# sloisel/MultiGridBarrier.jl

Measured on AMD Instinct MI355X. Metric: Newton iters/sec + wall-clock to converge, 2D P2 p-Laplace L=9, higher is better.
Workload: dtype f64

## Files before the change

multigridbarrier.jl_amd/csrc/mf_big_inv.hpp:

```cpp
#pragma once
#include "mf_device.hpp"

namespace mgbhip {
namespace {

constexpr int BIGI_THREADS = 1024;

#include "ldlt32.hpp"

__device__ __forceinline__ void block_ldlt32(double (*Dn)[NB + 1], double* dq, int nb, int tid, int32_t* __restrict__ status) {
    block_ldlt32_mfma(Dn, dq, nb, tid, status);
}
__device__ __forceinline__ void block_inverse32_sel(const double (*Ls)[NB + 1], double (*Wv)[NB + 1], double (*Tm)[17], int tid) {
    block_inverse32_mfma(Ls, Wv, Tm, tid);
}

__device__ __forceinline__ void block0_to_slot(double (*Dn)[NB + 1], double (*Wv)[NB + 1], double (*Tm)[17], double* dq, int nb,
                                               int tid, int32_t* __restrict__ status, double* __restrict__ slot) {
    block_ldlt32(Dn, dq, nb, tid, status);
    block_inverse32_sel(Dn, Wv, Tm, tid);
    for (int i = tid; i < NB * NB; i += 256) {
        const int rr = i % NB, c = i / NB;
        if (rr >= c && rr < nb) slot[rr + NB * c] = (rr == c) ? dq[rr] : Wv[rr][c];
    }
}

__device__ __forceinline__ void slice_transform(double (*P)[ST + 1], double (*Pout)[ST + 1], double (*P2)[ST + 1],
                                                const double (*Wv)[NB + 1], const double* rd, int lane, int wave) {
    const int fr = lane & 15, fk = lane >> 4;
    const int rr = 16 * wave + fr;
    double4_t acc0 = {0.0, 0.0, 0.0, 0.0}, acc1 = {0.0, 0.0, 0.0, 0.0};
#pragma unroll
    for (int kk = 0; kk < NB / 4; ++kk) {
        const double a = P[4 * kk + fk][rr];
        if (kk < 4) acc0 = __builtin_amdgcn_mfma_f64_16x16x4f64(Wv[fr][4 * kk + fk], a, acc0, 0, 0, 0);
        acc1 = __builtin_amdgcn_mfma_f64_16x16x4f64(Wv[16 + fr][4 * kk + fk], a, acc1, 0, 0, 0);
    }
#pragma unroll
    for (int r = 0; r < 4; ++r) {
        const int q0 = fk + 4 * r, q1 = 16 + fk + 4 * r;
        Pout[q0][rr] = acc0[r];
        Pout[q1][rr] = acc1[r];
        if (P2) {
            P2[q0][rr] = acc0[r] * rd[q0];
            P2[q1][rr] = acc1[r] * rd[q1];
        }
    }
}

#ifdef MGB_STEP_PROBE
#define PROBE(i) do { __builtin_amdgcn_sched_barrier(0); __builtin_amdgcn_s_waitcnt(0); if (is_la && blockIdx.y == 0 && tid == 0 && j0 == 64 && gridDim.y == 1 && F.k > 400) g_probe[i] = wall_clock64(); if (!is_la && blockIdx.x == 0 && blockIdx.y == 0 && tid == 0 && j0 == 64 && gridDim.y == 1 && F.k > 400) g_probe[16 + i] = wall_clock64(); __builtin_amdgcn_s_waitcnt(0); __builtin_amdgcn_sched_barrier(0); } while (0)
#else
#define PROBE(i) do { } while (0)
#endif

__global__ __launch_bounds__(256, 3) void mf_big_step(const FrontDev* __restrict__ fr, int32_t first, int j0,
                                                   double* __restrict__ arena, double* __restrict__ dscr,
                                                   double* __restrict__ dvec, int32_t* __restrict__ status,
                                                   int do_diag) {
    __shared__ double Wv[NB][NB + 1];
    __shared__ double Dn[NB][NB + 1];
    __shared__ double Tm[16][17];
    __shared__ double dq[NB], rdq[NB];
    __shared__ double Pa[NB][ST + 1];
    __shared__ double Pb[NB][ST + 1];
    const FrontDev F = fr[first + blockIdx.y];
    const int m = F.m, k = F.k;
    if (j0 >= k) return;
    const int nb = min(NB, k - j0);
    const int j1 = j0 + nb;
    const int T = (m - j1 + ST - 1) / ST;
    const int tid = threadIdx.x, lane = tid & 63, wave = tid >> 6;
    double* W = arena + F.F_off;
    double* slot = dscr + ((int64_t)blockIdx.y * 2 + ((j0 / NB) & 1)) * (NB * NB);
    const bool is_la = blockIdx.x == gridDim.x - 1;
    int ti = 0, tj = 0;
    if (!is_la) {
        const int lin = blockIdx.x;
        ti = (int)((sqrt(8.0 * lin + 1.0) - 1.0) * 0.5);
        while ((ti + 1) * (ti + 2) / 2 <= lin) ++ti;
        while (ti * (ti + 1) / 2 > lin) --ti;
        tj = lin - ti * (ti + 1) / 2;
        if (ti >= T) return;
    }
    const bool look = j1 < k;
    const int nbn = look ? min(NB, k - j1) : 0;
    const int rbase = is_la ? j1 : j1 + ti * ST, cbase = j1 + tj * ST;
    PROBE(0);
#ifdef MGB_STEP_PROBE
    if (is_la && blockIdx.y == 0 && tid == 0 && j0 == 64 && gridDim.y == 1 && F.k > 400) g_probe[34] = clock64();
#endif
    const int fr16 = lane & 15, fk = lane >> 4;

    double pa[NB * ST / 256], pb[NB * ST / 256];
#pragma unroll
    for (int u = 0; u < NB * ST / 256; ++u) {
        const int i = tid + 256 * u, rr = i % ST, q = i / ST;
        const int r = rbase + rr, c = cbase + rr;
        const bool rin = is_la ? (rr < nbn) : (r < m);
        pa[u] = (q < nb && rin) ? W[r + (int64_t)(j0 + q) * m] : 0.0;
        pb[u] = (!is_la && ti != tj && q < nb && c < m) ? W[c + (int64_t)(j0 + q) * m] : 0.0;
    }
    double cw[4][4];
    if (!is_la) {
#pragma unroll
        for (int tb = 0; tb < 4; ++tb)
#pragma unroll
            for (int r = 0; r < 4; ++r) {
                const int row = rbase + 16 * wave + fr16, col = cbase + 16 * tb + fk + 4 * r;
                cw[tb][r] = (row < m && col < m && row >= col) ? W[row + (int64_t)col * m] : 0.0;
            }
    } else {
#pragma unroll
        for (int t = 0; t < 4; ++t) {
            const int i = tid + 256 * t, rr = i % NB, c = i / NB;
            cw[0][t] = (look && rr >= c && rr < nbn) ? W[(j1 + rr) + (int64_t)(j1 + c) * m] : 0.0;
        }
    }
    if (do_diag) {
        for (int i = tid; i < NB * NB; i += 256) {
            const int rr = i % NB, c = i / NB;
            Dn[rr][c] = (rr >= c && rr < nb) ? W[(j0 + rr) + (int64_t)(j0 + c) * m] : 0.0;
        }
        __syncthreads();
        block_ldlt32(Dn, dq, nb, tid, is_la ? status : nullptr);
        block_inverse32_sel(Dn, Wv, Tm, tid);
    } else {
        for (int i = tid; i < NB * NB; i += 256) {
            const int rr = i % NB, c = i / NB;
            const double v = (rr >= c && rr < nb) ? slot[rr + NB * c] : 0.0;
            Wv[rr][c] = (rr > c) ? v : (rr == c ? 1.0 : 0.0);
            if (rr == c) dq[rr] = (rr < nb) ? v : 1.0;
        }
    }
#pragma unroll
    for (int u = 0; u < NB * ST / 256; ++u) {
        const int i = tid + 256 * u, rr = i % ST, q = i / ST;
        Pa[q][rr] = pa[u];
        Pb[q][rr] = pb[u];
    }
    __syncthreads();
    PROBE(1);
    if (tid < NB) rdq[tid] = 1.0 / dq[tid];
    if (is_la ? T == 0 : blockIdx.x == 0) {
        {
            const int rt = wave & 1, ct = wave >> 1;
            if (ct <= rt) {
                double4_t accm = {0.0, 0.0, 0.0, 0.0};
#pragma unroll
                for (int kk = 0; kk < NB / 4; ++kk) {
                    const int kq = 4 * kk + fk;
                    accm = __builtin_amdgcn_mfma_f64_16x16x4f64(kq < nb ? Wv[kq][16 * ct + fr16] / dq[kq] : 0.0, Wv[kq][16 * rt + fr16], accm, 0, 0, 0);
                }
#pragma unroll
                for (int r = 0; r < 4; ++r) {
                    const int row = 16 * rt + fr16, col = 16 * ct + fk + 4 * r;
                    if (row < nb && col < row) W[(j0 + col) + (int64_t)(j0 + row) * m] = accm[r];
                    else if (row < nb && col == row) dvec[F.idx_off + j0 + row] = accm[r];
                }
            }
        }
    }
    if (is_la && !look) return;
    __syncthreads();
    PROBE(2);
    if (is_la) {
        if (wave < 2) slice_transform(Pa, Pa, Pb, Wv, rdq, lane, wave);
        __syncthreads();
        PROBE(3);
        {
            const int rt = wave & 1, ct = wave >> 1;
            double4_t accd = {0.0, 0.0, 0.0, 0.0};
#pragma unroll
            for (int kk = 0; kk < NB / 4; ++kk)
                accd = __builtin_amdgcn_mfma_f64_16x16x4f64(Pb[4 * kk + fk][16 * ct + fr16], Pa[4 * kk + fk][16 * rt + fr16],
                                                            accd, 0, 0, 0);
#pragma unroll
            for (int r = 0; r < 4; ++r) {
                const int rr = 16 * rt + fr16, c = 16 * ct + fk + 4 * r;
                Dn[rr][c] = -accd[r];
            }
        }
        __syncthreads();
#pragma unroll
        for (int t = 0; t < 4; ++t) {
            const int i = tid + 256 * t, rr = i % NB, c = i / NB;
            Dn[rr][c] = (rr >= c && rr < nbn) ? cw[0][t] + Dn[rr][c] : 0.0;
        }
        __syncthreads();
        double* nslot = dscr + ((int64_t)blockIdx.y * 2 + ((j1 / NB) & 1)) * (NB * NB);
        PROBE(4);
#ifdef MGB_STEP_PROBE
        double sv[4];
        for (int t = 0; t < 4; ++t) { const int i = tid + 256 * t; sv[t] = Dn[i % NB][i / NB]; }
        __syncthreads();
        __builtin_amdgcn_sched_barrier(0);
        if (is_la && blockIdx.y == 0 && tid == 0 && j0 == 64 && gridDim.y == 1 && F.k > 400) { g_probe[32] = clock64(); g_probe[36] = wall_clock64(); }
        __builtin_amdgcn_sched_barrier(0);
        block_ldlt32(Dn, dq, nbn, tid, nullptr);
        __builtin_amdgcn_sched_barrier(0);
        if (is_la && blockIdx.y == 0 && tid == 0 && j0 == 64 && gridDim.y == 1 && F.k > 400) { g_probe[33] = clock64(); g_probe[37] = wall_clock64(); }
        __builtin_amdgcn_sched_barrier(0);
        for (int t = 0; t < 4; ++t) { const int i = tid + 256 * t; Dn[i % NB][i / NB] = sv[t]; }
        __syncthreads();
        __builtin_amdgcn_sched_barrier(0);
        if (is_la && blockIdx.y == 0 && tid == 0 && j0 == 64 && gridDim.y == 1 && F.k > 400) { g_probe[38] = clock64(); g_probe[44] = wall_clock64(); }
        __builtin_amdgcn_sched_barrier(0);
#endif
        block_ldlt32(Dn, dq, nbn, tid, status);
#ifdef MGB_STEP_PROBE
        __builtin_amdgcn_sched_barrier(0);
        if (is_la && blockIdx.y == 0 && tid == 0 && j0 == 64 && gridDim.y == 1 && F.k > 400) { g_probe[39] = clock64(); g_probe[45] = wall_clock64(); }
        __builtin_amdgcn_sched_barrier(0);
#endif
        PROBE(5);
        block_inverse32_sel(Dn, Wv, Tm, tid);
        PROBE(6);
        for (int i = tid; i < NB * NB; i += 256) {
            const int rr = i % NB, c = i / NB;
            if (rr >= c && rr < nbn) nslot[rr + NB * c] = (rr == c) ? dq[rr] : Wv[rr][c];
        }
        PROBE(7);
#ifdef MGB_STEP_PROBE
        if (is_la && blockIdx.y == 0 && tid == 0 && j0 == 64 && gridDim.y == 1 && F.k > 400) g_probe[35] = clock64();
#endif
        return;
    }
    if (ti == tj) {
        slice_transform(Pa, Pa, Pb, Wv, rdq, lane, wave);
    } else {
        slice_transform(Pa, Pa, nullptr, Wv, rdq, lane, wave);
        {
            const int rr = 16 * wave + fr16;
            double4_t acc0 = {0.0, 0.0, 0.0, 0.0}, acc1 = {0.0, 0.0, 0.0, 0.0};
#pragma unroll
            for (int kk = 0; kk < NB / 4; ++kk) {
                const double a = Pb[4 * kk + fk][rr];
                if (kk < 4) acc0 = __builtin_amdgcn_mfma_f64_16x16x4f64(Wv[fr16][4 * kk + fk], a, acc0, 0, 0, 0);
                acc1 = __builtin_amdgcn_mfma_f64_16x16x4f64(Wv[16 + fr16][4 * kk + fk], a, acc1, 0, 0, 0);
            }
#pragma unroll
            for (int r = 0; r < 4; ++r) {
                const int q0 = fk + 4 * r, q1 = 16 + fk + 4 * r;
                Pb[q0][rr] = acc0[r] * rdq[q0];
                Pb[q1][rr] = acc1[r] * rdq[q1];
            }
        }
    }
    __syncthreads();
    PROBE(3);
    double4_t acc[4];
#pragma unroll
    for (int tb = 0; tb < 4; ++tb) acc[tb] = double4_t{0.0, 0.0, 0.0, 0.0};
#pragma unroll
    for (int kk = 0; kk < NB / 4; ++kk) {
        const double s = Pa[4 * kk + fk][16 * wave + fr16];
#pragma unroll
        for (int tb = 0; tb < 4; ++tb) {
            if (ti == tj && tb > wave) continue;
            acc[tb] = __builtin_amdgcn_mfma_f64_16x16x4f64(Pb[4 * kk + fk][16 * tb + fr16], s, acc[tb], 0, 0, 0);
        }
    }
    const int nskip = (blockIdx.x == 0 && look) ? nbn : 0;
#pragma unroll
    for (int tb = 0; tb < 4; ++tb)
#pragma unroll
        for (int r = 0; r < 4; ++r) {
            const int row = rbase + 16 * wave + fr16, col = cbase + 16 * tb + fk + 4 * r;
            if (row < m && col < m && row >= col && !(row - j1 < nskip && col - j1 < nskip))
                W[row + (int64_t)col * m] = cw[tb][r] - acc[tb][r];
        }
    PROBE(4);
}

__global__ __launch_bounds__(256) void mf_tri_pack(int m, const double* __restrict__ F, double* __restrict__ packed, int unpack,
                                                   double* __restrict__ Fout) {
    const int c = blockIdx.x;
    if (c >= m) return;
    const int64_t base = (int64_t)c * m - ((int64_t)c * (c - 1)) / 2;
    for (int r = c + threadIdx.x; r < m; r += 256) {
        if (unpack) Fout[r + (int64_t)c * m] = packed[base + (r - c)];
        else packed[base + (r - c)] = F[r + (int64_t)c * m];
    }
}

__global__ __launch_bounds__(256) void mf_big_diag0(const FrontDev* __restrict__ fr, int32_t first,
                                                    const double* __restrict__ arena, double* __restrict__ dscr,
                                                    int32_t* __restrict__ status) {
    __shared__ double Wv[NB][NB + 1];
    __shared__ double Dn[NB][NB + 1];
    __shared__ double Tm[16][17];
    __shared__ double dq[NB];
    const FrontDev F = fr[first + blockIdx.x];
    const int m = F.m, nb = min(NB, F.k), tid = threadIdx.x;
    const double* W = arena + F.F_off;
    for (int i = tid; i < NB * NB; i += 256) {
        const int rr = i % NB, c = i / NB;
        Dn[rr][c] = (rr >= c && rr < nb) ? W[rr + (int64_t)c * m] : 0.0;
    }
    __syncthreads();
    block0_to_slot(Dn, Wv, Tm, dq, nb, tid, status, dscr + (int64_t)blockIdx.x * 2 * (NB * NB));
}

__global__ __launch_bounds__(BIGI_THREADS) void mf_fwd_inv(const FrontDev* __restrict__ fr, int32_t first,
                                                           const int32_t* __restrict__ front_idx,
                                                           const int64_t* __restrict__ ug_ptr,
                                                           const int64_t* __restrict__ ug_src,
                                                           const double* __restrict__ arena,
                                                           const double* __restrict__ dvec,
                                                           const double* __restrict__ b, double* __restrict__ y,
                                                           double* __restrict__ uvec) {
    extern __shared__ double sh[];
#ifdef MGB_STEP_PROBE
#define FP(i) do { if (threadIdx.x == 0 && gridDim.x > 150) { const long long _t = wall_clock64(); if (blockIdx.x == 0) g_probe[48 + i] = _t; if (i == 0) atomicMin((unsigned long long*)&g_probe[56], (unsigned long long)_t); if (i == 5) { atomicMax((unsigned long long*)&g_probe[57], (unsigned long long)_t); atomicAdd((unsigned long long*)&g_probe[58], (unsigned long long)(_t - g_probe[56])); } } } while (0)
#else
#define FP(i) do { } while (0)
#endif
    FP(0);
    const FrontDev F = fr[first + blockIdx.x];
    const int m = F.m, k = F.k;
    const int tid = threadIdx.x, nt = BIGI_THREADS;
    double* tl = sh;
    double* Ml = sh + ((m + 1) & ~1);
    double* uq = Ml + NB * (NB + 1);
    double* part = uq + 2 * NB;
    const int32_t* idx = front_idx + F.idx_off;
    const double* Fm = arena + F.F_off;
    const double* dv = dvec + F.idx_off;
    {
        const int64_t* up = ug_ptr + F.ug_off;
        for (int j = tid; j < m; j += nt) {
            double v = (j < k) ? b[idx[j]] : 0.0;
            const int64_t e1 = up[j + 1];
            for (int64_t e = up[j]; e < e1; e += 4) {
                double a[4];
#pragma unroll
                for (int u = 0; u < 4; ++u) a[u] = (e + u < e1) ? uvec[ug_src[e + u]] : 0.0;
#pragma unroll
                for (int u = 0; u < 4; ++u) v += a[u];
            }
            tl[j] = v;
        }
    }
    const int wa = tid % NB, wb = tid / NB;
    {
        const double w0 = (wa < wb && wb < k) ? Fm[wa + (int64_t)wb * m] : 0.0;
        if (wa < wb) { Ml[wb * (NB + 1) + wa] = w0; Ml[wa * (NB + 1) + wb] = w0; }
        if (tid < NB) Ml[tid * (NB + 1) + tid] = (tid < k) ? dv[tid] : 0.0;
    }
    __syncthreads();
    FP(1);
    for (int j0 = 0; j0 < k; j0 += NB) {
        const int nb = min(NB, k - j0), j1 = j0 + nb;
        const int jn = j0 + NB;
        const double wnext = (wa < wb && jn + wb < k) ? Fm[(jn + wa) + (int64_t)(jn + wb) * m] : 0.0;
// ... 219 lines not shown
                    }
                }
            }
        }
        {
            const int q = tid >> 5, c = tid & 31;
            double ph = Ml[q * (NB + 1) + c] * (c < nb ? gl[j0 + c] : 0.0);
            ph += quad_perm_f64<0xB1>(ph);
            ph += quad_perm_f64<0x4E>(ph);
            ph += quad_perm_f64<0x124>(ph);
            ph += quad_perm_f64<0x128>(ph);
            ph += __shfl_xor(ph, 16, 32);
            if (c == 0) zq[q] = (q < nb) ? tl[j0 + q] - ph : 0.0;
        }
        if (j0 == 256) BP(5);
        __syncthreads();
        if (j0 == 256) BP(6);
        if (tid < nb) x[il[j0 + tid]] = zq[tid];
        if (wa < wb) { Ml[wb * (NB + 1) + wa] = wnext; Ml[wa * (NB + 1) + wb] = wnext; }
        if (tid < NB) Ml[tid * (NB + 1) + tid] = dnext;
        double zr[8];
#pragma unroll
        for (int t = 0; t < 4; ++t) {
            zr[2 * t] = zq[2 * cp + 8 * t];
            zr[2 * t + 1] = zq[2 * cp + 8 * t + 1];
        }
#pragma unroll
        for (int ps = 0; ps < 2; ++ps) {
            const int q = cq + ps * CPP;
            if (q < j0) {
                double v = 0.0;
#pragma unroll
                for (int t = 0; t < 4; ++t) v += pa[ps][t].a * zr[2 * t] + pa[ps][t].b * zr[2 * t + 1];
                v += quad_perm_f64<0xB1>(v);
                v += quad_perm_f64<0x4E>(v);
                if (cp == 0) gl[q] += v;
            }
        }
        for (int q = cq + 2 * CPP; q - cq < j0; q += CPP) {
            const double* Aq = Fm + (int64_t)min(q, j0 - 1) * m + j0 + 2 * cp;
            D2 a[4];
#pragma unroll
            for (int t = 0; t < 4; ++t) {
                if (nb == NB) a[t] = *reinterpret_cast<const D2*>(Aq + 8 * t);
                else {
                    const int o = 2 * cp + 8 * t;
                    a[t].a = Aq[min(o, nb - 1) - 2 * cp];
                    a[t].b = Aq[min(o + 1, nb - 1) - 2 * cp];
                }
            }
            double v = 0.0;
#pragma unroll
            for (int t = 0; t < 4; ++t) v += a[t].a * zr[2 * t] + a[t].b * zr[2 * t + 1];
            v += quad_perm_f64<0xB1>(v);
            v += quad_perm_f64<0x4E>(v);
            if (cp == 0 && q < j0) gl[q] += v;
        }
        if (j0 == 256) BP(7);
        __syncthreads();
    }
    BP(9);
}

__global__ __launch_bounds__(BIGI_THREADS) void mf_bwd_inv(const FrontDev* __restrict__ fr, int32_t first,
                                                           const int32_t* __restrict__ front_idx,
                                                           const double* __restrict__ arena,
                                                           const double* __restrict__ dvec,
                                                           const double* __restrict__ y, double* __restrict__ x) {
    bwd_inv_front<false>(fr, first, blockIdx.x, front_idx, arena, dvec, y, x, nullptr, 0, nullptr);
}
__global__ __launch_bounds__(BIGI_THREADS) void mf_bwd_inv_split(const FrontDev* __restrict__ fr, int32_t first,
                                                                 const int32_t* __restrict__ front_idx,
                                                                 const double* __restrict__ arena,
                                                                 const double* __restrict__ dvec,
                                                                 const double* __restrict__ y, double* __restrict__ x,
                                                                 double* gscr, int gstride, uint32_t* cnt) {
    bwd_inv_front<true>(fr, first, blockIdx.y, front_idx, arena, dvec, y, x, gscr, gstride, cnt);
}

inline void launch_big_diag0(const FactorArgs& a, const MfLaunch& L, int nfronts) {
    hipLaunchKernelGGL(mf_big_diag0, dim3(nfronts), dim3(256), 0, a.st, a.fr, L.first, a.arena, a.dscr, a.status);
}
inline void launch_inv_steps(const FactorArgs& a, const MfLaunch& L, int nfronts, bool diag_in_step0) {
    for (int j0 = 0; j0 < L.max_k; j0 += NB) {
        const int rem = L.max_m - j0;
        const int T = std::max(0, (rem - 1 + ST - 1) / ST);
        const dim3 gs(T * (T + 1) / 2 + 1, nfronts);
        hipLaunchKernelGGL(mf_big_step, gs, dim3(256), 0, a.st, a.fr, L.first, j0, a.arena, a.dscr, a.dvec, a.status,
                           (j0 == 0 && diag_in_step0) ? 1 : 0);
    }
}

inline void launch_tri_pack(int m, double* F, double* packed, bool unpack, hipStream_t st) {
    hipLaunchKernelGGL(mf_tri_pack, dim3(m), dim3(256), 0, st, m, unpack ? (const double*)nullptr : F, packed, unpack ? 1 : 0,
                       unpack ? F : (double*)nullptr);
}

inline size_t fwd_inv_lds(int max_m) {
    return (size_t)(((max_m + 1) & ~1) + NB * (NB + 1) + 2 * NB + BIGI_THREADS) * sizeof(double);
}
inline size_t bwd_inv_lds(int max_m, int max_k) {
    return (size_t)(((max_m + 1) & ~1) + ((max_k + 1) & ~1) + NB * (NB + 1) + 2 * NB + (max_m + 1) / 2) * sizeof(double);
}
inline void launch_fwd_inv(const SolveArgs& a, const MfLaunch& L) {
    hipLaunchKernelGGL(mf_fwd_inv, dim3(L.count), dim3(BIGI_THREADS), fwd_inv_lds(L.max_m), a.st, a.fr, L.first, a.front_idx,
                       a.ug_ptr, a.ug_src, a.arena, a.dvec, a.b, a.y, a.uvec);
}
inline void launch_bwd_inv(const SolveArgs& a, const MfLaunch& L) {
    const int S = a.bwd_cnt ? bwd_inv_split(L.count, L.max_k, L.max_m) : 1;
    if (S > 1) {
        hipLaunchKernelGGL(mf_bwd_inv_split, dim3(S, L.count), dim3(BIGI_THREADS), bwd_inv_lds(L.max_m, L.max_k), a.st, a.fr, L.first,
                           a.front_idx, a.arena, a.dvec, a.y, a.x, a.bwd_g, (int)bwd_split_stride(L.max_k), a.bwd_cnt);
        return;
    }
    hipLaunchKernelGGL(mf_bwd_inv, dim3(L.count), dim3(BIGI_THREADS), bwd_inv_lds(L.max_m, L.max_k), a.st, a.fr, L.first,
                       a.front_idx, a.arena, a.dvec, a.y, a.x);
}

}
}
```

multigridbarrier.jl_amd/csrc/mf_launch_plan.hpp:

```cpp
#pragma once
#include <algorithm>
#include <cstdint>
#include <cstdlib>
#include <vector>

#include "host_util.hpp"
#include "mf_analysis.hpp"

namespace mgbhip {

struct MfLaunch {
    int32_t first, count;
    int32_t cls;
    int32_t max_m, max_k;
    int32_t max_child = 0;
    bool tiny = false;
    bool wave = false;
    bool inv = false;
    bool iface = false;
    int32_t grec_first = -1;
};

constexpr int BIG_INV_MAX_M = 7000;
constexpr int GATHER_MAX_CHILD = 8;
constexpr int BIG_DIAG0_MIN_COUNT = 24;

struct MfSwitches {
    bool no_geo;
    bool old_big;
    bool merge_groups;
    bool packed_leaves;
    bool wave_small;
    int64_t inv_min_n;
    int64_t wave_min_n;
    bool gather_lds_maps;
    int gather_ct;
    bool bwd_split;
    int small_threads;
    bool border_launches;
    static MfSwitches from_env() {
        auto num = [](const char* name, long long dflt) { const char* e = getenv(name); return e ? atoll(e) : dflt; };
        return {env_on("MGBHIP_NO_GEO"), env_on("MGBHIP_OLD_BIG"), !env_on("MGBHIP_NO_MERGE_GROUPS"), !env_on("MGBHIP_NO_PACKED_LEAVES"),
                !env_on("MGBHIP_NO_WAVE_SMALL"), num("MGBHIP_INV_MIN_N", 1024), num("MGBHIP_WAVE_MIN_N", 0),
                env_on("MGBHIP_GATHER_LDS_MAPS"), (int)num("MGBHIP_GATHER_CT", 0), num("MGBHIP_BWD_SPLIT", 1) != 0,
                (int)num("MGBHIP_SMALL_THREADS", 0), env_on("MGBHIP_BORDER_LAUNCHES")};
    }
};

using LevelLaunches = std::vector<std::vector<MfLaunch>>;

inline MfLaunch launch_of_range(const MfPlan& plan, MfLaunch L, int32_t first, int32_t count) {
    L.first = first; L.count = count;
    L.max_m = 0; L.max_k = 0; L.max_child = 0;
    for (int32_t t = first; t < first + count; ++t) {
        L.max_m = std::max(L.max_m, plan.fronts[t].m);
        L.max_k = std::max(L.max_k, plan.fronts[t].k);
        L.max_child = std::max(L.max_child, plan.fronts[t].nchild);
    }
    return L;
}

inline void merge_straggler_groups(const MfPlan& plan, std::vector<MfLaunch>& G) {
    auto absorb = [&](size_t into, size_t from) {
        MfLaunch& A = G[into];
        const MfLaunch& B = G[from];
        A.first = B.first;
        A.count += B.count;
        A.max_k = std::max(A.max_k, B.max_k);
        A.max_child = std::max(A.max_child, B.max_child);
        G.erase(G.begin() + (long)from);
    };
    if (G.size() >= 2 && G.back().cls == 0 && G.back().inv) {
        int64_t lds_count = 0;
        bool ok = true;
        for (size_t g = 0; g + 1 < G.size(); ++g) { lds_count += G[g].count; ok = ok && !G[g].tiny && plan.fronts[G[g].first].m > 32; }
        if (ok && lds_count <= G.back().count)
            while (G.size() >= 2) absorb(G.size() - 1, G.size() - 2);
    }
    for (size_t g = 0; g + 1 < G.size();) {
        const bool next_lds = G[g + 1].cls != 0;
        if (next_lds && !G[g].tiny && (G[g].count < 256 || 4 * (int64_t)G[g].count < G[g + 1].count)) absorb(g + 1, g);
        else ++g;
    }
}

inline void split_interface_front(const MfPlan& plan, LevelLaunches& levels, bool inv_allowed) {
    const int32_t q = plan.iface_front;
    for (auto& G : levels) {
        for (size_t g = 0; g < G.size(); ++g) {
            const MfLaunch L = G[g];
            if (q < L.first || q >= L.first + L.count) continue;
            std::vector<MfLaunch> out;
            if (q > L.first) out.push_back(launch_of_range(plan, L, L.first, q - L.first));
            MfLaunch I = launch_of_range(plan, L, q, 1);
            I.cls = 0; I.tiny = false; I.wave = false; I.iface = true;
            I.inv = (I.max_m <= BIG_INV_MAX_M && inv_allowed);
            out.push_back(I);
            if (q + 1 < L.first + L.count) out.push_back(launch_of_range(plan, L, q + 1, L.first + L.count - q - 1));
            G.erase(G.begin() + (long)g);
            G.insert(G.begin() + (long)g, out.begin(), out.end());
            break;
        }
    }
}

inline bool only_small_children(const MfPlan& plan, const MfLaunch& L) {
    for (int32_t q = L.first; q < L.first + L.count; ++q) {
        const Front& f = plan.fronts[q];
        for (int32_t c = 0; c < f.nchild; ++c) {
            const Front& ch = plan.fronts[plan.children[f.child_off + c]];
            if ((ch.m - ch.k) * (ch.m - ch.k) > 64) return false;
        }
    }
    return true;
}

inline LevelLaunches classify_launches(const MfPlan& plan, int32_t lds_cap, bool inv_ok, const MfSwitches& sw) {
    static const int32_t classes[] = {16, 32, 48, 64, 88, 128};
    const bool inv_allowed = inv_ok && !sw.old_big && plan.n >= sw.inv_min_n;
    const int32_t nlev = (int32_t)plan.level_ptr.size() - 1;
    LevelLaunches levels(nlev);
    for (int32_t l = 0; l < nlev; ++l) {
        int32_t i = plan.level_ptr[l];
        const int32_t end = plan.level_ptr[l + 1];
        while (i < end) {
            const int32_t m = plan.fronts[i].m;
            int32_t cls = 0;
            for (int32_t c : classes)
// ... 77 lines not shown
    return (L.iface || L.count >= BIG_DIAG0_MIN_COUNT) ? MF_B0_DIAG0 : MF_B0_STEP0;
}
inline int backward_small_kmax(const MfLaunch& L) { return L.max_k <= 8 ? 8 : (L.max_k <= 16 ? 16 : 0); }

inline size_t factor_small_lds(int cls) {
    return (size_t)((cls >= 88 ? cls * (cls + 1) / 2 : cls * cls) + 8 * cls) * sizeof(double);
}
constexpr int SMALL_STATIC_LDS = 2112;
constexpr int CU_LDS_BYTES = 160 * 1024;
constexpr int SMALL_FILL_WAVES = 24;
inline int factor_small_threads(const MfLaunch& L, int compute_units, int forced = 0) {
    if (L.cls <= 16) return 64;
    if (L.cls <= 32) return 128;
    if (forced == 256 || forced == 512 || forced == 1024) return forced;
    const int64_t cu = std::max(compute_units, 1);
    const int64_t fit = std::max<int64_t>(1, CU_LDS_BYTES / (int64_t)(factor_small_lds(L.cls) + SMALL_STATIC_LDS));
    const int64_t per_cu = std::min(fit, ((int64_t)L.count + cu - 1) / cu);
    int threads = 256;
    while (threads < 1024 && per_cu * (2 * threads / 64) <= SMALL_FILL_WAVES) threads *= 2;
    return threads;
}
static_assert(16 - 1 <= 64 && 32 - 1 <= 128 && 128 - 1 <= 256, "mf_factor_small solves one panel row per thread");

constexpr int GATHER_MIN_WGS = 768;
inline int big_gather_ct(const MfLaunch& L, int forced) {
    if (forced == 8 || forced == 16 || forced == 32) return forced;
    int ct = 8;
    while (ct < 32 && (int64_t)L.count * ((L.max_m + 2 * ct - 1) / (2 * ct)) >= GATHER_MIN_WGS) ct *= 2;
    return ct;
}

constexpr int BWD_SPLIT_MAX = 16;
constexpr int BWD_SPLIT_CUS = 256;
constexpr int BWD_SPLIT_COLS = 64;
constexpr int BWD_THIN_BOUNDARY = 8;
inline int bwd_inv_split(int32_t count, int32_t max_k, int32_t max_m) {
    if (count < 1 || max_m - max_k <= BWD_THIN_BOUNDARY) return 1;
    return std::max(1, std::min({BWD_SPLIT_MAX, BWD_SPLIT_CUS / count, (max_k + BWD_SPLIT_COLS - 1) / BWD_SPLIT_COLS}));
}
inline int32_t bwd_split_stride(int32_t max_k) { return (max_k + 1) & ~1; }
inline void bwd_split_scratch(const LevelLaunches& solves, int64_t out[2]) {
    out[0] = out[1] = 0;
    for (auto& lev : solves)
        for (auto& L : lev) {
            if (L.count == 0 || L.cls || !L.inv || bwd_inv_split(L.count, L.max_k, L.max_m) == 1) continue;
            out[0] = std::max<int64_t>(out[0], L.count);
            out[1] = std::max<int64_t>(out[1], (int64_t)L.count * bwd_split_stride(L.max_k));
        }
}

struct GatherRec {
    int64_t map_off;
    int64_t base[GATHER_MAX_CHILD];
    int32_t ld[GATHER_MAX_CHILD];
    int32_t bs[GATHER_MAX_CHILD];
};

inline void build_gather_maps(const MfPlan& plan, LevelLaunches& levels, std::vector<GatherRec>& recs, std::vector<int32_t>& gmap) {
    recs.clear();
    gmap.clear();
    for (auto& lev : levels)
        for (auto& L : lev) {
            L.grec_first = -1;
            if (L.count == 0 || big_assembly_kind(L) != MF_ASM_GATHER) continue;
            L.grec_first = (int32_t)recs.size();
            for (int32_t q = L.first; q < L.first + L.count; ++q) {
                const Front& f = plan.fronts[q];
                GatherRec R{};
                R.map_off = (int64_t)gmap.size();
                gmap.resize(gmap.size() + (size_t)f.nchild * (size_t)f.m, -1);
                for (int32_t c = 0; c < f.nchild; ++c) {
                    const Front& ch = plan.fronts[plan.children[f.child_off + c]];
                    R.base[c] = ch.F_off + (int64_t)ch.k * ch.m + ch.k;
                    R.ld[c] = ch.m;
                    R.bs[c] = ch.m - ch.k;
                    int32_t* mp = gmap.data() + R.map_off + (int64_t)c * f.m;
                    for (int32_t j = 0; j < ch.m - ch.k; ++j) mp[plan.rel[ch.rel_off + j]] = j;
                }
                recs.push_back(R);
            }
        }
}

constexpr int MF_LAUNCH_ROW = 16;
inline int64_t launch_rows(const LevelLaunches& levels, const LevelLaunches& solves, bool leaf_packed, bool robust,
                           int32_t* out, int64_t cap) {
    int64_t n = 0;
    for (size_t l = 0; l < levels.size(); ++l) {
        int32_t bwd = 0;
        for (auto& S : solves[l])
            if (S.cls && !S.tiny) { const int km = backward_small_kmax(S); bwd = km == 8 ? MF_BWD_K8 : (km == 16 ? MF_BWD_K16 : MF_BWD_GENERAL); }
        for (auto& L : levels[l]) {
            if (n < cap && out) {
                const bool inv = L.inv && !robust;
                int32_t* r = out + n * MF_LAUNCH_ROW;
                r[0] = (int32_t)l; r[1] = L.first; r[2] = L.count; r[3] = L.cls; r[4] = L.max_m; r[5] = L.max_k; r[6] = L.max_child;
                r[7] = L.tiny; r[8] = L.wave; r[9] = inv; r[10] = L.iface; r[11] = L.tiny && leaf_packed;
                r[12] = big_assembly_kind(L); r[13] = big_block0_kind(L, inv); r[14] = (L.cls && !L.tiny) ? bwd : (int32_t)MF_BWD_NA; r[15] = 0;
            }
            ++n;
        }
    }
    return n;
}

}
```

multigridbarrier.jl_amd/csrc/mf_numeric.hip:

```cpp
#include <hip/hip_runtime.h>

#include <cstdio>

#include <algorithm>
#include <cstdlib>

#include "../../include/mgbhip.h"
#include "mf_solver.hpp"
#include "mf_device.hpp"
#include "mf_small.hpp"
#include "mf_big_subst.hpp"
#include "mf_big_inv.hpp"
#include "mf_big_assemble.hpp"

namespace mgbhip {

namespace {

int32_t query_lds_cap() {
    if (hipFuncSetAttribute((const void*)mf_factor_small<8, true>, hipFuncAttributeMaxDynamicSharedMemorySize,
                            (int)factor_small_lds(128)) == hipSuccess)
        return 128;
    (void)hipGetLastError();
    return 88;
// ... 88 lines not shown
    static StageTimers& timers_or_dummy(StageTimers* t) {
        static const bool on = env_on("MGBHIP_LEVEL_TIMING");
        return (t && on) ? *t : g_dummy_timers;
    }
    LevelScope(StageTimers* t, const char* sweep, int level)
        : scope(timers_or_dummy(t), (snprintf(nm, sizeof(nm), "%s_lv%02d", sweep, level), nm)) {}
};

}

void MfSolver::upload_plan(hipStream_t st) {
    d_front_idx.upload(plan.front_idx, st);
    d_children.upload(plan.children, st);
    d_rel.upload(plan.rel, st);
    d_a_src.upload(plan.a_src, st);
    d_a_colptr.upload(plan.a_colptr, st);
    d_arena.alloc((size_t)std::max<int64_t>(plan.arena_doubles, 1));
    d_uvec.alloc((size_t)std::max<int64_t>(plan.uvec_doubles, 1));
    d_y.alloc((size_t)plan.n + 1);
    y_zero = y_border_one = status_zero = leaf_zero = false;
    d_bx.alloc((size_t)plan.n + 1);
    d_xx.alloc((size_t)plan.n + 1);
    {
        const double one = 1.0;
        d_one.upload(&one, 1, st);
        MGB_HIP_CHECK(hipStreamSynchronize(st));
    }
    d_tbig.alloc(plan.front_idx.size() ? plan.front_idx.size() : 1);
    d_tsol.alloc(plan.front_idx.size() ? plan.front_idx.size() : 1);
    d_dvec.alloc(plan.front_idx.size() ? plan.front_idx.size() : 1);
    d_status.alloc(2);
    d_status.zero(st);
}

void MfSolver::analyze(int64_t n, const int32_t* rowptr, const int32_t* colidx, hipStream_t st,
                       const double* coords, int dim, bool protect_peeled, const int32_t* top, int64_t ntop) {
    const MfSwitches sw = MfSwitches::from_env();
    MfOptions opt;
    opt.protect_peeled = protect_peeled;
    opt.top = top;
    opt.ntop = ntop;
    opt.border = true;
    mf_analyze(n, rowptr, colidx, opt, plan, sw.no_geo ? nullptr : coords, dim);
    const int32_t nf = (int32_t)plan.fronts.size();
    std::vector<FrontDev> fd(nf);
    for (int32_t i = 0; i < nf; ++i) {
        const Front& f = plan.fronts[i];
        fd[i] = FrontDev{f.k, f.m, f.nchild, f.a_cnt, f.F_off, f.idx_off, f.u_off, f.child_off, f.rel_off, f.a_off, f.acol_off, -1, 0, 0};
    }
    upload_plan(st);

    lds_cap = query_lds_cap();
    const bool inv_ok = !sw.old_big && query_inv_optin();
    level_launches = classify_launches(plan, lds_cap, inv_ok, sw);
    level_solves = merge_level_solves(level_launches);
    uses_inv = false;
    const std::vector<char> on_big_path = fronts_on_big_path(plan, level_launches);
    int32_t max_big = 1;
    for (auto& lev : level_launches)
        for (auto& L : lev) {
            uses_inv = uses_inv || L.inv;
            if (!L.cls) max_big = std::max(max_big, L.count);
        }
    d_dscr.alloc((size_t)max_big * 2 * NB * NB);
    {
        int64_t need[2] = {0, 0};
        if (sw.bwd_split) bwd_split_scratch(level_solves, need);
        if (need[0] == 0) { d_bwd_g.release(); d_bwd_cnt.release(); }
        else {
            d_bwd_g.alloc((size_t)need[1]);
            d_bwd_cnt.alloc((size_t)need[0]);
            d_bwd_cnt.zero(st);
        }
    }

    std::vector<int64_t> ug_ptr, ug_src;
    build_gather_lists(plan, on_big_path, fd, ug_ptr, ug_src);
    leaf_packed = sw.packed_leaves && pack_leaf_fronts(plan, level_launches, on_big_path, fd);
    d_ug_ptr.upload(ug_ptr, st);
    d_ug_src.upload(ug_src, st);
    std::vector<GatherRec> grec;
    std::vector<int32_t> gmap;
    if (!sw.gather_lds_maps) build_gather_maps(plan, level_launches, grec, gmap);
    gather_ct = sw.gather_ct;
    small_threads = sw.small_threads;
    {
        int dev = 0, cus = 0;
        MGB_HIP_CHECK(hipGetDevice(&dev));
        MGB_HIP_CHECK(hipDeviceGetAttribute(&cus, hipDeviceAttributeMultiprocessorCount, dev));
        compute_units = std::max(cus, 1);
    }
    border_launches = sw.border_launches;
    {
        const int32_t nlev = (int32_t)plan.level_ptr.size() - 1;
        border_alone = false;
        if (plan.border && nlev >= 2 && plan.level_ptr[nlev] - plan.level_ptr[nlev - 1] == 1) {
            const Front& f = plan.fronts[plan.level_ptr[nlev - 1]];
            border_alone = f.m == 1 && f.k == 1 && plan.front_idx[f.idx_off] == (int32_t)plan.n;
        }
    }
    border_skipped = false;
    carried_x = nullptr;
    if (grec.empty()) { d_grec.release(); d_gmap.release(); }
    else { d_grec.upload(grec, st); d_gmap.upload(gmap, st); }
    d_fronts.upload(fd, st);
    h_fronts = fd;
    h_a_dst = remap_a_dst(plan, level_launches);
    d_a_dst.upload(h_a_dst, st);
    if (debug_level() >= 2) dump_plan(plan, level_launches);
    analyzed = true;
    MGB_HIP_CHECK(hipStreamSynchronize(st));
}

void MfSolver::set_direct_map(const int32_t* value_map, int64_t nnz, int64_t tail_base, hipStream_t st) {
    std::vector<int32_t> as(plan.a_src.size());
    for (size_t t = 0; t < as.size(); ++t) {
        const int64_t src = plan.a_src[t];
        const int64_t v = src < nnz ? (int64_t)value_map[src] : tail_base + (src - nnz);
        MGB_REQUIRE(v < (int64_t)INT32_MAX, "direct value index exceeds 32 bits");
        as[t] = (int32_t)v;
    }
    d_a_src_direct.upload(as, st);
    MGB_HIP_CHECK(hipStreamSynchronize(st));
}

bool MfSolver::skips_border() const {
    return analyzed && border_alone && !border_launches && !robust && plan.iface_front < 0;
}

void MfSolver::factor(const double* d_values, hipStream_t st, StageTimers* timers, bool direct, bool condensed, double* carried_x_np1) {
    MGB_REQUIRE(!direct || d_a_src_direct.n > 0, "MfSolver::factor: no direct value map");
    MGB_REQUIRE(!condensed || (direct && condensed_ok), "MfSolver::factor: condensed leaves are not enabled");
    MGB_REQUIRE(analyzed, "MfSolver::factor before analyze");
    const FactorArgs a{condensed ? d_fronts_c.p : d_fronts.p, d_children.p, d_rel.p,
                       condensed ? d_a_src_c.p : (direct ? d_a_src_direct.p : d_a_src.p), condensed ? d_a_dst_c.p : d_a_dst.p,
                       condensed ? d_a_colptr_c.p : d_a_colptr.p, d_values, d_arena.p, d_dscr.p, d_dvec.p, d_status.p, st,
                       d_grec.n ? d_grec.p : nullptr, d_gmap.p, gather_ct, small_threads, compute_units};
    if (timers) timers->begin("factor");
    factored_inv = !robust;
    border_skipped = carried_x_np1 != nullptr && skips_border();
    carried_x = border_skipped ? carried_x_np1 : nullptr;
    const int border_level = (int)level_launches.size() - 1;
    if (!status_zero) MGB_HIP_CHECK(hipMemsetAsync(d_status.p, 0, sizeof(int32_t), st));
    status_zero = false;
    factored_condensed = condensed;
    int lvno = -1;
    for (auto& lev : level_launches) {
        if (border_skipped && lvno + 1 == border_level) break;
        LevelScope lvscope(timers, "fac", ++lvno);
        for (auto& L : lev) {
            if (L.count == 0) continue;
            if (condensed && lvno == 0) continue;
            if (L.tiny) launch_factor_tiny(a, L);
            else if (L.wave && L.cls <= 32) launch_factor_wave<32>(a, L);
            else if (L.wave) launch_factor_wave<48>(a, L);
            else if (L.cls) launch_factor_small(a, L);
            else {
                const bool inv = L.inv && !robust;
                const MfBlock0 b0 = big_block0_kind(L, inv);
                MGB_REQUIRE(!L.iface || (bool)iface_reduce, "MfSolver: interface front without a reduction hook");
                launch_big_assemble(a, L, b0 == MF_B0_GATHER);
                if (L.iface) {
                    const Front& fi = plan.fronts[L.first];
                    const int64_t tri = (int64_t)fi.m * (fi.m + 1) / 2;
                    d_ifpack.ensure((size_t)tri);
                    launch_tri_pack(fi.m, d_arena.p + fi.F_off, d_ifpack.p, false, st);
                    iface_reduce(d_ifpack.p, tri);
                    launch_tri_pack(fi.m, d_arena.p + fi.F_off, d_ifpack.p, true, st);
                }
                if (inv) {
                    if (b0 == MF_B0_DIAG0) launch_big_diag0(a, L, L.count);
                    launch_inv_steps(a, L, L.count, b0 == MF_B0_STEP0);
                } else
                    launch_subst_steps(a, L, L.count);
            }
        }
    }
    MGB_HIP_CHECK(hipGetLastError());
    if (timers) timers->end();
}

void MfSolver::solve(const double* d_b, double* d_x, hipStream_t st, StageTimers* timers) {
    MGB_REQUIRE(analyzed, "MfSolver::solve before analyze");
    MGB_REQUIRE(!border_skipped, "MfSolver::solve on factors that carry a Newton right-hand side");
    if (timers) timers->begin("trisolve");
    const size_t n = (size_t)plan.n;
    MGB_HIP_CHECK(hipMemcpyAsync(d_bx.p, d_b, n * sizeof(double), hipMemcpyDeviceToDevice, st));
    MGB_HIP_CHECK(hipMemsetAsync(d_bx.p + n, 0, sizeof(double), st));
    forward_pass(d_bx.p, st, timers);
    backward_pass(d_xx.p, st, timers);
    MGB_HIP_CHECK(hipMemcpyAsync(d_x, d_xx.p, n * sizeof(double), hipMemcpyDeviceToDevice, st));
    MGB_HIP_CHECK(hipGetLastError());
    if (timers) timers->end();
}

void MfSolver::solve_border(double* d_x_np1, hipStream_t st, StageTimers* timers) {
    MGB_REQUIRE(analyzed, "MfSolver::solve_border before analyze");
    if (timers) timers->begin("trisolve");
    const size_t n = (size_t)plan.n;
    if (!y_zero) {
        MGB_HIP_CHECK(hipMemsetAsync(d_y.p, 0, n * sizeof(double), st));
        y_zero = true;
    }
    if (!y_border_one) {
        MGB_HIP_CHECK(hipMemcpyAsync(d_y.p + n, d_one.p, sizeof(double), hipMemcpyDeviceToDevice, st));
        y_border_one = true;
    }
    if (border_skipped && d_x_np1 != carried_x)
        MGB_HIP_CHECK(hipMemcpyAsync(d_x_np1 + n, d_one.p, sizeof(double), hipMemcpyDeviceToDevice, st));
    backward_pass(d_x_np1, st, timers, border_skipped);
    MGB_HIP_CHECK(hipGetLastError());
    if (timers) timers->end();
}

void MfSolver::forward_pass(const double* d_b, hipStream_t st, StageTimers* timers) {
    y_border_one = false;
    y_zero = false;
    const SolveArgs a = solve_args(d_b, nullptr, st);
    int lvno = -1;
    for (auto& lev : level_solves) {
// ... 152 lines not shown
```

multigridbarrier.jl_amd/csrc/mf_solver.hpp:

```cpp
#pragma once
#include <functional>

#include "common.hpp"
#include "mf_analysis.hpp"
#include "mf_launch_plan.hpp"
#include "kernels.hpp"

namespace mgbhip {

struct FrontDev {
    int32_t k, m, nchild, a_cnt;
    int64_t F_off, idx_off, u_off, child_off, rel_off, a_off, acol_off;
    int64_t ug_off;
    int32_t packed;
    int32_t pad_;
};

struct FactorArgs {
    const FrontDev* fr;
    const int32_t *children, *rel, *a_src, *a_dst, *a_colptr;
    const double* values;
    double *arena, *dscr, *dvec;
    int32_t* status;
    hipStream_t st;
    const GatherRec* grec;
    const int32_t* gmap;
    int gather_ct;
    int small_threads;
    int compute_units;
};
struct SolveArgs {
    const FrontDev* fr;
    const int32_t *front_idx, *children, *rel;
    const int64_t *ug_ptr, *ug_src;
    const double *arena, *dvec;
    const double* b;
    double *y, *x, *uvec, *tbig, *tsol;
    hipStream_t st;
    double* bwd_g;
    uint32_t* bwd_cnt;
};

class MfSolver {
   public:
    MfPlan plan;
    void analyze(int64_t n, const int32_t* rowptr, const int32_t* colidx, hipStream_t st,
                 const double* coords = nullptr, int dim = 0, bool protect_peeled = false,
                 const int32_t* top = nullptr, int64_t ntop = 0);
    std::function<void(double*, int64_t)> iface_reduce;
    void factor(const double* d_values, hipStream_t st, StageTimers* timers, bool direct = false, bool condensed = false,
                double* carried_x = nullptr);
    bool skips_border() const;
    bool enable_condensed(int64_t N, int P, const int32_t* ucol, int64_t slack0, int64_t nnz, int64_t tail_base, hipStream_t st);
    bool condensed_ready() const { return condensed_ok; }
    bool leaves_packed() const { return leaf_packed; }
    const LeafDesc* leaf_desc() const { return d_leaf_desc.p; }
    double* arena() { return d_arena.p; }
    int32_t* leaf_status() { return d_status.p + 1; }
    const int32_t* status_flags() const { return d_status.p; }
    int32_t* status_flags_rw() { return d_status.p; }
    void flags_cleared() { status_zero = true; leaf_zero = true; }
    bool leaf_flag_zero() const { return leaf_zero; }
    void leaf_flag_used() { leaf_zero = false; }
    void set_direct_map(const int32_t* value_map, int64_t nnz, int64_t tail_base, hipStream_t st);
    bool has_direct_map() const { return d_a_src_direct.n > 0; }
    void solve(const double* d_b, double* d_x, hipStream_t st, StageTimers* timers);
    void solve_border(double* d_x_np1, hipStream_t st, StageTimers* timers);
    void chain_stats(double* out8) const;
    int64_t launches(int32_t* out, int64_t cap) const;
    int status(hipStream_t st);
    void status_async(int32_t* h_dst, hipStream_t st) const;
    static int status_from(const int32_t* flags2, bool with_leaves) {
        return (flags2[0] || (with_leaves && flags2[1])) ? MGBHIP_ERR_NOT_SPD : MGBHIP_OK;
    }
    bool factored_condensed = false;
    bool analyzed = false;
    bool robust = false;
    bool has_inverse_path() const { return uses_inv; }
    bool factored_inv = false;

   private:
    void upload_plan(hipStream_t st);
    SolveArgs solve_args(const double* d_b, double* d_x, hipStream_t st) const {
        return {d_fronts.p, d_front_idx.p, d_children.p, d_rel.p, d_ug_ptr.p, d_ug_src.p, d_arena.p, d_dvec.p, d_b, d_y.p, d_x,
                d_uvec.p, d_tbig.p, d_tsol.p, st, d_bwd_g.p, d_bwd_cnt.n ? d_bwd_cnt.p : nullptr};
    }
    void forward_pass(const double* d_b_np1, hipStream_t st, StageTimers* timers);
    void backward_pass(double* d_x_np1, hipStream_t st, StageTimers* timers, bool without_border = false);
    DevBuf<double> d_bx, d_xx, d_one;
    DevBuf<FrontDev> d_fronts;
    DevBuf<int32_t> d_front_idx, d_children, d_rel, d_a_src, d_a_src_direct, d_a_dst, d_a_colptr;
    DevBuf<GatherRec> d_grec;
    DevBuf<int32_t> d_gmap;
    DevBuf<int64_t> d_ug_ptr, d_ug_src;
    DevBuf<double> d_arena, d_uvec, d_y, d_tbig, d_tsol, d_dscr, d_dvec;
    DevBuf<double> d_ifpack;
    DevBuf<int32_t> d_status;
    DevBuf<double> d_bwd_g;
    DevBuf<uint32_t> d_bwd_cnt;
    bool condensed_ok = false;
    bool leaf_packed = false;
    std::vector<FrontDev> h_fronts;
    std::vector<int32_t> h_a_dst;
    DevBuf<FrontDev> d_fronts_c;
    DevBuf<int32_t> d_a_src_c, d_a_dst_c, d_a_colptr_c;
    DevBuf<LeafDesc> d_leaf_desc;
    std::vector<std::vector<MfLaunch>> level_launches;
    std::vector<std::vector<MfLaunch>> level_solves;
    int gather_ct = 0;
    int small_threads = 0;
    int compute_units = 1;
    bool border_launches = false;
    bool border_alone = false;
    bool border_skipped = false;
    const double* carried_x = nullptr;
    int32_t lds_cap = 88;
    bool uses_inv = false;
    bool y_border_one = false;
    bool y_zero = false;
    bool status_zero = false, leaf_zero = false;
};

}
```

Before: 715.0.

## Fold small row-tails into diagonal tiles of big-front LDLT step kernel

```diff
diff --git a/multigridbarrier.jl_amd/csrc/mf_big_inv.hpp b/multigridbarrier.jl_amd/csrc/mf_big_inv.hpp
--- a/multigridbarrier.jl_amd/csrc/mf_big_inv.hpp
+++ b/multigridbarrier.jl_amd/csrc/mf_big_inv.hpp
@@ -54,10 +54,11 @@
 #define PROBE(i) do { } while (0)
 #endif
 
-__global__ __launch_bounds__(256, 3) void mf_big_step(const FrontDev* __restrict__ fr, int32_t first, int j0,
-                                                   double* __restrict__ arena, double* __restrict__ dscr,
-                                                   double* __restrict__ dvec, int32_t* __restrict__ status,
-                                                   int do_diag) {
+template <bool TAIL>
+__device__ __forceinline__ void big_step_front(const FrontDev* __restrict__ fr, int32_t first, int j0,
+                                               double* __restrict__ arena, double* __restrict__ dscr,
+                                               double* __restrict__ dvec, int32_t* __restrict__ status,
+                                               int do_diag) {
     __shared__ double Wv[NB][NB + 1];
     __shared__ double Dn[NB][NB + 1];
     __shared__ double Tm[16][17];
@@ -69,7 +70,8 @@
     if (j0 >= k) return;
     const int nb = min(NB, k - j0);
     const int j1 = j0 + nb;
-    const int T = (m - j1 + ST - 1) / ST;
+    const StepTiles tiles = step_tiles(m, j1, TAIL);
+    const int T = tiles.T;
     const int tid = threadIdx.x, lane = tid & 63, wave = tid >> 6;
     double* W = arena + F.F_off;
     double* slot = dscr + ((int64_t)blockIdx.y * 2 + ((j0 / NB) & 1)) * (NB * NB);
@@ -84,6 +86,7 @@
         if (ti >= T) return;
     }
     const bool look = j1 < k;
+    if (is_la && !look && T > 0) return;
     const int nbn = look ? min(NB, k - j1) : 0;
     const int rbase = is_la ? j1 : j1 + ti * ST, cbase = j1 + tj * ST;
     PROBE(0);
@@ -141,6 +144,17 @@
     }
     __syncthreads();
     PROBE(1);
+    const bool fold = TAIL && !is_la && ti == tj && tiles.tail > 0;
+    const int r0 = j1 + T * ST, trow = r0 + fr16;
+    const bool tin = fold && fr16 < tiles.tail;
+    double at[NB / 4];
+    if (TAIL) {
+#pragma unroll
+        for (int kk = 0; kk < NB / 4; ++kk) {
+            const int q = 4 * kk + fk;
+            at[kk] = (tin && q < nb) ? W[trow + (int64_t)(j0 + q) * m] : 0.0;
+        }
+    }
     if (tid < NB) rdq[tid] = 1.0 / dq[tid];
     if (is_la ? T == 0 : blockIdx.x == 0) {
         {
@@ -271,6 +285,55 @@
                 W[row + (int64_t)col * m] = cw[tb][r] - acc[tb][r];
         }
     PROBE(4);
+    if (fold) {
+        double ct[4];
+#pragma unroll
+        for (int r = 0; r < 4; ++r) ct[r] = tin ? W[trow + (int64_t)(cbase + 16 * wave + fk + 4 * r) * m] : 0.0;
+        double4_t s0 = {0.0, 0.0, 0.0, 0.0}, s1 = {0.0, 0.0, 0.0, 0.0};
+#pragma unroll
+        for (int kk = 0; kk < NB / 4; ++kk) {
+            if (kk < 4) s0 = __builtin_amdgcn_mfma_f64_16x16x4f64(Wv[fr16][4 * kk + fk], at[kk], s0, 0, 0, 0);
+            s1 = __builtin_amdgcn_mfma_f64_16x16x4f64(Wv[16 + fr16][4 * kk + fk], at[kk], s1, 0, 0, 0);
+        }
+        const double sk[NB / 4] = {s0[0], s0[1], s0[2], s0[3], s1[0], s1[1], s1[2], s1[3]};
+        double4_t acct = {0.0, 0.0, 0.0, 0.0};
+#pragma unroll
+        for (int kk = 0; kk < NB / 4; ++kk)
+            acct = __builtin_amdgcn_mfma_f64_16x16x4f64(Pb[4 * kk + fk][16 * wave + fr16], sk[kk], acct, 0, 0, 0);
+#pragma unroll
+        for (int r = 0; r < 4; ++r)
+            if (tin) W[trow + (int64_t)(cbase + 16 * wave + fk + 4 * r) * m] = ct[r] - acct[r];
+        if (tj == T - 1 && wave == 0) {
+            double cc[4];
+#pragma unroll
+            for (int r = 0; r < 4; ++r) {
+                const int ccol = r0 + fk + 4 * r;
+                cc[r] = (tin && ccol <= trow) ? W[trow + (int64_t)ccol * m] : 0.0;
+            }
+            double4_t accc = {0.0, 0.0, 0.0, 0.0};
+#pragma unroll
+            for (int kk = 0; kk < NB / 4; ++kk)
+                accc = __builtin_amdgcn_mfma_f64_16x16x4f64(sk[kk] * rdq[4 * kk + fk], sk[kk], accc, 0, 0, 0);
+#pragma unroll
+            for (int r = 0; r < 4; ++r) {
+                const int ccol = r0 + fk + 4 * r;
+                if (tin && ccol <= trow) W[trow + (int64_t)ccol * m] = cc[r] - accc[r];
+            }
+        }
+    }
+}
+
+__global__ __launch_bounds__(256, 3) void mf_big_step(const FrontDev* __restrict__ fr, int32_t first, int j0,
+                                                   double* __restrict__ arena, double* __restrict__ dscr,
+                                                   double* __restrict__ dvec, int32_t* __restrict__ status,
+                                                   int do_diag) {
+    big_step_front<false>(fr, first, j0, arena, dscr, dvec, status, do_diag);
+}
+__global__ __launch_bounds__(256, 3) void mf_big_step_tail(const FrontDev* __restrict__ fr, int32_t first, int j0,
+                                                        double* __restrict__ arena, double* __restrict__ dscr,
+                                                        double* __restrict__ dvec, int32_t* __restrict__ status,
+                                                        int do_diag) {
+    big_step_front<true>(fr, first, j0, arena, dscr, dvec, status, do_diag);
 }
 
 __global__ __launch_bounds__(256) void mf_tri_pack(int m, const double* __restrict__ F, double* __restrict__ packed, int unpack,
@@ -656,12 +719,13 @@
     hipLaunchKernelGGL(mf_big_diag0, dim3(nfronts), dim3(256), 0, a.st, a.fr, L.first, a.arena, a.dscr, a.status);
 }
 inline void launch_inv_steps(const FactorArgs& a, const MfLaunch& L, int nfronts, bool diag_in_step0) {
-    for (int j0 = 0; j0 < L.max_k; j0 += NB) {
-        const int rem = L.max_m - j0;
-        const int T = std::max(0, (rem - 1 + ST - 1) / ST);
-        const dim3 gs(T * (T + 1) / 2 + 1, nfronts);
-        hipLaunchKernelGGL(mf_big_step, gs, dim3(256), 0, a.st, a.fr, L.first, j0, a.arena, a.dscr, a.dvec, a.status,
-                           (j0 == 0 && diag_in_step0) ? 1 : 0);
+    static_assert(NB == STEP_COLS && ST == STEP_TILE, "step_tiles (mf_launch_plan.hpp) tiles for this kernel");
+    MGB_REQUIRE(L.step_first >= 0, "launch_inv_steps: a launch without step grids");
+    const StepGrid* grid = a.step_grid + L.step_first;
+    for (int j0 = 0; j0 < L.max_k; j0 += NB, ++grid) {
+        const dim3 gs(grid->tiles + 1, nfronts);
+        hipLaunchKernelGGL(grid->tail ? mf_big_step_tail : mf_big_step, gs, dim3(256), 0, a.st, a.fr, L.first, j0, a.arena, a.dscr,
+                           a.dvec, a.status, (j0 == 0 && diag_in_step0) ? 1 : 0);
     }
 }
 
diff --git a/multigridbarrier.jl_amd/csrc/mf_launch_plan.hpp b/multigridbarrier.jl_amd/csrc/mf_launch_plan.hpp
--- a/multigridbarrier.jl_amd/csrc/mf_launch_plan.hpp
+++ b/multigridbarrier.jl_amd/csrc/mf_launch_plan.hpp
@@ -19,6 +19,7 @@
     bool inv = false;
     bool iface = false;
     int32_t grec_first = -1;
+    int32_t step_first = -1;
 };
 
 constexpr int BIG_INV_MAX_M = 7000;
@@ -38,12 +39,13 @@
     bool bwd_split;
     int small_threads;
     bool border_launches;
+    bool step_tail;
     static MfSwitches from_env() {
         auto num = [](const char* name, long long dflt) { const char* e = getenv(name); return e ? atoll(e) : dflt; };
         return {env_on("MGBHIP_NO_GEO"), env_on("MGBHIP_OLD_BIG"), !env_on("MGBHIP_NO_MERGE_GROUPS"), !env_on("MGBHIP_NO_PACKED_LEAVES"),
                 !env_on("MGBHIP_NO_WAVE_SMALL"), num("MGBHIP_INV_MIN_N", 1024), num("MGBHIP_WAVE_MIN_N", 0),
                 env_on("MGBHIP_GATHER_LDS_MAPS"), (int)num("MGBHIP_GATHER_CT", 0), num("MGBHIP_BWD_SPLIT", 1) != 0,
-                (int)num("MGBHIP_SMALL_THREADS", 0), env_on("MGBHIP_BORDER_LAUNCHES")};
+                (int)num("MGBHIP_SMALL_THREADS", 0), env_on("MGBHIP_BORDER_LAUNCHES"), num("MGBHIP_STEP_TAIL", 1) != 0};
     }
 };
 
@@ -287,6 +289,51 @@
         }
 }
 
+#ifdef __HIPCC__
+#define MGB_PLAN_HD __host__ __device__
+#else
+#define MGB_PLAN_HD
+#endif
+constexpr int STEP_COLS = 32;
+constexpr int STEP_TILE = 64;
+constexpr int STEP_TAIL_MAX = 16;
+struct StepTiles {
+    int T;
+    int tail;
+};
+MGB_PLAN_HD inline StepTiles step_tiles(int m, int j1, bool fold) {
+    const int rem = m - j1;
+    if (rem <= 0) return {0, 0};
+    const int tail = rem % STEP_TILE;
+    if (fold && tail >= 1 && tail <= STEP_TAIL_MAX && rem >= STEP_TILE) return {rem / STEP_TILE, tail};
+    return {(rem + STEP_TILE - 1) / STEP_TILE, 0};
+}
+struct StepGrid {
+    int32_t tiles;
+    int32_t tail;
+};
+inline StepGrid step_grid(const Front* fronts, int32_t count, int j0, bool fold) {
+    StepGrid g{0, 0};
+    for (int32_t t = 0; t < count; ++t) {
+        const int m = fronts[t].m, k = fronts[t].k;
+        if (j0 >= k) continue;
+        const StepTiles s = step_tiles(m, j0 + std::min(STEP_COLS, k - j0), fold);
+        g.tiles = std::max(g.tiles, s.T * (s.T + 1) / 2);
+        g.tail = g.tail || s.tail > 0;
+    }
+    return g;
+}
+inline void build_step_grids(const MfPlan& plan, LevelLaunches& levels, bool fold, std::vector<StepGrid>& grids) {
+    grids.clear();
+    for (auto& lev : levels)
+        for (auto& L : lev) {
+            L.step_first = -1;
+            if (L.count == 0 || L.cls) continue;
+            L.step_first = (int32_t)grids.size();
+            for (int j0 = 0; j0 < L.max_k; j0 += STEP_COLS) grids.push_back(step_grid(plan.fronts.data() + L.first, L.count, j0, fold));
+        }
+}
+
 constexpr int MF_LAUNCH_ROW = 16;
 inline int64_t launch_rows(const LevelLaunches& levels, const LevelLaunches& solves, bool leaf_packed, bool robust,
                            int32_t* out, int64_t cap) {
diff --git a/multigridbarrier.jl_amd/csrc/mf_numeric.hip b/multigridbarrier.jl_amd/csrc/mf_numeric.hip
--- a/multigridbarrier.jl_amd/csrc/mf_numeric.hip
+++ b/multigridbarrier.jl_amd/csrc/mf_numeric.hip
@@ -194,6 +194,7 @@
     std::vector<GatherRec> grec;
     std::vector<int32_t> gmap;
     if (!sw.gather_lds_maps) build_gather_maps(plan, level_launches, grec, gmap);
+    build_step_grids(plan, level_launches, sw.step_tail, step_grids);
     gather_ct = sw.gather_ct;
     small_threads = sw.small_threads;
     {
@@ -247,7 +248,7 @@
     const FactorArgs a{condensed ? d_fronts_c.p : d_fronts.p, d_children.p, d_rel.p,
                        condensed ? d_a_src_c.p : (direct ? d_a_src_direct.p : d_a_src.p), condensed ? d_a_dst_c.p : d_a_dst.p,
                        condensed ? d_a_colptr_c.p : d_a_colptr.p, d_values, d_arena.p, d_dscr.p, d_dvec.p, d_status.p, st,
-                       d_grec.n ? d_grec.p : nullptr, d_gmap.p, gather_ct, small_threads, compute_units};
+                       d_grec.n ? d_grec.p : nullptr, d_gmap.p, gather_ct, small_threads, compute_units, step_grids.data()};
     if (timers) timers->begin("factor");
     factored_inv = !robust;
     border_skipped = carried_x_np1 != nullptr && skips_border();
diff --git a/multigridbarrier.jl_amd/csrc/mf_solver.hpp b/multigridbarrier.jl_amd/csrc/mf_solver.hpp
--- a/multigridbarrier.jl_amd/csrc/mf_solver.hpp
+++ b/multigridbarrier.jl_amd/csrc/mf_solver.hpp
@@ -28,6 +28,7 @@
     int gather_ct;
     int small_threads;
     int compute_units;
+    const StepGrid* step_grid;
 };
 struct SolveArgs {
     const FrontDev* fr;
@@ -107,6 +108,7 @@
     DevBuf<LeafDesc> d_leaf_desc;
     std::vector<std::vector<MfLaunch>> level_launches;
     std::vector<std::vector<MfLaunch>> level_solves;
+    std::vector<StepGrid> step_grids;
     int gather_ct = 0;
     int small_threads = 0;
     int compute_units = 1;
```

New measurement: 713.2. About the same (-0.2%).
